# leonlang/simple_raytracer

Measured on AMD Instinct MI355X. Metric: Mrays/sec (primary+shadow) at 1920x1080; max per-pixel |dRGB| vs CPU ref, higher is better.
Workload: dtype f32; 1 GPU; ground_bunny: stanford-bunny (69,451 tris) over a ground slab, BVH + slab-AABB, 1920x1080, 1 light sample(s) [BASELINE.json configs[2]]; nodes=24216, tris=69463, parallelism=1 GPU, launch=hipGraph replay, 4 stream(s), pipeline=k_trace_nq+k_shade_tile

## Files before the change

simple_raytracer_amd/csrc/srt_hip.hip:

```cpp
#include <hip/hip_runtime.h>

#include <cfloat>
#include <cmath>
#include <cstdio>
#include <cstdlib>
#include <cstring>
#include <algorithm>
#include <array>
#include <atomic>
#include <deque>
#include <map>
#include <memory>
#include <new>
#include <thread>
#include <type_traits>
#include <vector>

#include "../../include/srt.h"
#include "srt_device.h"

using namespace srt;

#include "srt_kernels.h"
#include "srt_packet.h"
// ... 945 lines not shown

uint64_t srt_scene_device_bytes(const srt_scene* s) { return s ? s->bytes : 0; }
const char* srt_scene_pipeline(const srt_scene* s) { return s ? s->pipeline : ""; }
double srt_scene_overlap_estimate(const srt_scene* s) { return s ? s->rec->overlap : 0.; }

enum Variant : uint32_t {
    V_SHIPPED = 0,
    V_REFERENCE = 1,
    V_TRI_QUEUE = 2,
    V_NQ_TINY = 3,
    V_NQ_EXACT = 4,
    V_NQ_8X4 = 5,
    V_NQ_TINY_FILTER = 6,
    V_UNFUSED = 10,
    V_FUSED_5_WAVES = 11,
    V_FUSED_ROOTS_AGAIN = 12,
    V_FUSED_HALF = 13,
    V_FUSED_HALF_TINY = 14,
    V_FUSED_HALF_1024 = 15,
    V_FUSED_HALF_32_RAYS = 16,
    V_FUSED_64_RAYS = 17,
    V_XCD_ROWS = 18,
    V_FUSED_HALF_6_WAVES = 19,
    V_CHUNKED = 20,
    V_NQ_PK = 21,
    V_PK_PK = 22,
    V_PK_NQ = 23,
    V_NO_PACKET = 24,
    V_PK_WINDOWS = 25,
    V_COARSE_GRID = 27,
    V_TRACE_SHADE = 28,
    V_PK_ENTRY_ORDER = 29,
    V_FUSED_HALF_8_WAVES = 30,
    V_CAMERA_PK = 35,
    V_ROUND2_FORM = 40,
    V_ALL_WIDE = 41,
    V_ALL_NARROW = 42,
    V_LANE_ORDER = 43,
    V_GENERAL_SHADE = 44,
    V_ROOT_LOOP = 45,
    V_NO_UNION_BOX = 46,
    V_WIDE_STEP_COUNTERS = 47,
    V_HIT_6_WAVES = 53,
    V_FUSED_6_WAVES = 54,
    V_PK_AHEAD = 55,
    V_PK_AHEAD_SKIP = 56,
    V_PK_PLAIN = 57,
    V_PK_CLOCKS = 58,
    V_FUSED_FOUR_WAVES = 59,
    V_SHADOW_PLAIN_ROWS = 62,
    V_EXACT_TONE = 63,
    V_FULL_GRID = 64,
    V_HALF_7_WAVES = 65,
    V_HALF_8_WAVES_256 = 66,
};
static inline uint32_t variant_of(const srt_params* p) { return (p->flags >> 8) & 0xffu; }
static inline uint32_t variant_or_shipped(const srt_params* p) { const uint32_t v = variant_of(p); return v >= V_FULL_GRID && v <= V_HALF_8_WAVES_256 ? (uint32_t)V_SHIPPED : v; }
static inline bool shipped_choice(uint32_t v) {
    return v == V_SHIPPED || v == V_NO_PACKET || v == V_PK_WINDOWS || v == V_COARSE_GRID || v == V_PK_ENTRY_ORDER || v == V_CAMERA_PK ||
           (v >= V_ROUND2_FORM && v <= V_SHADOW_PLAIN_ROWS) || v == V_EXACT_TONE;
}

using RefHitFn = decltype(&k_closest_hit<false>);
using RefShadeFn = decltype(&k_shade<false>);
using QHitFn = decltype(&k_closest_hit_q<false>);
using NqHitFn = decltype(&k_closest_hit_nq<false, 512, 2, 2, true>);
using PkHitFn = decltype(&k_closest_hit_pk<false, true, false>);
using TraceFn = decltype(&k_trace_nq<false, 512, true, 7, 16>);
using TraceShadeFn = decltype(&k_trace_shade_nq<512, true, 6, 16>);
using ShadowPkFn = decltype(&k_shadow_pk<false, true, false>);
using ShadowNqFn = decltype(&k_shadow_nq<false, 512, true, 16, 6>);
using ShadeTileFn = decltype(&k_shade_tile<0>);
using TraceSpansFn = decltype(&k_trace_nq_spans<512, true, 7, 16>);
using ShadeTileSpansFn = decltype(&k_shade_tile_spans<0>);


enum BatchState { NOT_BATCHED, BATCH_FITS, BATCH_OTHER_SIZE };
enum Hold { HOLD_NONE, HOLD_FUSED, HOLD_PK };

struct SceneFacts {
    bool prefer_packet, int_shin, normals; double overlap; uint64_t bytes; uint32_t n_cu;
    uint32_t heavy_steps, pk_units, pk_take;
    uint32_t n_objects; const float* root_min; const float* root_max; uint32_t box_epoch;
};
static SceneFacts scene_facts(const srt_scene* s) {
    static const auto env = [](const char* name, uint32_t dflt) { const char* e = std::getenv(name); return e ? (uint32_t)std::strtoul(e, nullptr, 10) : dflt; };
    static const uint32_t heavy_steps = env("SRT_HEAVY_STEPS", 64u);
    static const uint32_t pk_units = env("SRT_PK_UNITS", 64u), pk_take = env("SRT_PK_TAKE", 4u);
    const bool boxes_known = s->rec->root_boxes_valid && !s->rec->boxes_change_in_replays;
    return SceneFacts{s->rec->prefer_packet, s->rec->int_shin, s->dev.tri_normals != nullptr, s->rec->overlap, s->bytes, (uint32_t)s->n_cu,
// ... 69 lines not shown
    if (holdable && (fused ? !pl.xcd_rows && !cam : pk_shadow)) {
        pl.hold = fused ? HOLD_FUSED : HOLD_PK;
        if (!fused) { pl.heavy_steps = f.heavy_steps; pl.pk_take = f.pk_take ? f.pk_take : 1u; pl.pk_units = 0u; }
        std::snprintf(pl.pipeline, sizeof(pl.pipeline), fused ? "k_trace_nq+k_shade_tile (batched)" : "k_closest_hit_nq+k_shadow_pk+k_shade_tile (batched)");
        return pl;
    }
    if (pk_shadow && v == V_SHIPPED && !count && !in_flight && batch == NOT_BATCHED) pl.heavy_steps = f.heavy_steps;

    #define NQ_HIT(CAP, TWL, THL, FILTER) do { \
        if (count) pl.nq_hit = &k_closest_hit_nq<true, CAP, TWL, THL, FILTER>; else pl.nq_hit = &k_closest_hit_nq<false, CAP, TWL, THL, FILTER>; \
        pl.grid_hit = dim3((wl + (2u << TWL) - 1) / (2u << TWL), (rows + (2u << THL) - 1) / (2u << THL)); } while (0)
    pl.grid_hit = grid8;
    switch (v) {
    case V_TRI_QUEUE:
        if (count) pl.q_hit = &k_closest_hit_q<true>; else pl.q_hit = &k_closest_hit_q<false>;
        pl.grid_hit = grid16; break;
    case V_NQ_TINY:        NQ_HIT(160, 2, 2, false); break;
    case V_NQ_EXACT:       NQ_HIT(512, 2, 2, false); break;
    case V_NQ_TINY_FILTER: NQ_HIT(160, 2, 2, true); break;
    case V_NQ_8X4:         NQ_HIT(1024, 3, 2, false); break;
    case V_UNFUSED:        NQ_HIT(512, 2, 2, true); break;
    default:
        if (pk_closest) {
            const bool xcd = pl.xcd_rows && !cam && !count;
            if (cam && count)  pl.pk_hit = &k_closest_hit_pk<true, true, false, true>;
            else if (cam)      pl.pk_hit = &k_closest_hit_pk<false, true, false, true>;
            else if (count)    pl.pk_hit = &k_closest_hit_pk<true, true, false>;
            else if (xcd)      pl.pk_hit = &k_closest_hit_pk<false, true, true>;
            else               pl.pk_hit = &k_closest_hit_pk<false, true, false>;
            pl.grid_hit = dim3((grid8.x + 1) / 2, xcd ? xcd_pad((grid8.y + 1) / 2) : (grid8.y + 1) / 2);
        } else if (fused && v == V_TRACE_SHADE && !count && !pl.xcd_rows && L < 64) {
            pl.trace_shade = &k_trace_shade_nq<512, true, 6, 16>;
        } else if (fused) {
            const bool half_tile = (v == V_SHIPPED && in_flight) || v == V_FUSED_HALF;
            const bool half_eight = (v == V_SHIPPED && in_flight && variant_of(p) != V_HALF_7_WAVES) || v == V_FUSED_HALF_8_WAVES;
            if (cam_nq)                        pl.trace = &k_trace_nq<false, 512, true, 5, 16, false, false, true>;
            else if (count)                    pl.trace = &k_trace_nq<true, 512, true, 5, 16>;
            else if (v == V_FUSED_5_WAVES)     pl.trace = &k_trace_nq<false, 512, true, 5, 16>;
            else if (v == V_FUSED_ROOTS_AGAIN) pl.trace = &k_trace_nq<false, 512, true, 6, 16, false, true>;
            else if (v == V_FUSED_64_RAYS)     pl.trace = &k_trace_nq<false, 512, true, 5, 64>;
            else if (v == V_FUSED_6_WAVES)     pl.trace = &k_trace_nq<false, 512, true, 6, 16>;
            else if (v == V_ALL_WIDE)          pl.trace = &k_trace_nq<false, 512, true, 6, 16, false, false, false, true>;
            else if (pl.xcd_rows)            { pl.trace = &k_trace_nq<false, 512, true, 6, 16, true>; pl.grid_hit.y = xcd_pad(grid8.y); }
            else if (v == V_FUSED_HALF_TINY) { pl.trace = &k_trace_nq_half<160, true, 6, 16>; pl.block_hit = 128; }
            else if (v == V_FUSED_HALF_1024) { pl.trace = &k_trace_nq_half<1024, true, 5, 16>; pl.block_hit = 128; }
            else if (v == V_FUSED_HALF_32_RAYS) { pl.trace = &k_trace_nq_half<512, true, 6, 32>; pl.block_hit = 128; }
            else if (v == V_FUSED_HALF_6_WAVES) { pl.trace = &k_trace_nq_half<512, true, 6, 16>; pl.block_hit = 128; }
            else if (half_eight && variant_of(p) == V_HALF_8_WAVES_256) { pl.trace = &k_trace_nq_half8<256, true, 16>; pl.block_hit = 128; }
            else if (half_eight)             { pl.trace = &k_trace_nq_half8<384, true, 16>; pl.block_hit = 128; }
            else if (half_tile)              { pl.trace = &k_trace_nq_half<512, true, 7, 16>; pl.block_hit = 128; }
            else                               pl.trace = &k_trace_nq<false, 512, true, 7, 16>;
        } else if (!count && v == V_COARSE_GRID) {
            pl.nq_hit = &k_closest_hit_nq<false, 512, 2, 2, true, true>;
            pl.grid_hit = dim3((grid8.x + 1) / 2, (grid8.y + 1) / 2);
        } else if (!count && v == V_ALL_WIDE) {
            pl.nq_hit = &k_closest_hit_nq<false, 512, 2, 2, true, false, true>;
        } else if (!count && v != V_HIT_6_WAVES) {
            pl.nq_hit = &k_closest_hit_nq<false, 512, 2, 2, true, false, false, 7>;
        } else {
            NQ_HIT(512, 2, 2, true);
        }
    }
    #undef NQ_HIT
    if (pk_shadow) {
        const uint64_t max_units = (uint64_t)n_tiles * 4u * 2u * ((L + 7) / 8);
        pl.grid_shadow = dim3((uint32_t)(max_units / 4 + 1 < (uint64_t)f.n_cu * 8 ? max_units / 4 + 1 : (uint64_t)f.n_cu * 8));
        if (count)                       pl.shadow_pk = &k_shadow_pk<true, true, false>;
        else if (v == V_PK_ENTRY_ORDER)  pl.shadow_pk = &k_shadow_pk<false, true, false, true>;
        else if (v == V_PK_AHEAD)        pl.shadow_pk = &k_shadow_pk<false, true, false, false, 1>;
        else if (v == V_PK_AHEAD_SKIP)   pl.shadow_pk = &k_shadow_pk<false, true, false, false, 2>;
        else if (pl.heavy_steps)         pl.shadow_pk = &k_shadow_pk<false, true, false, false, 0, true>;
        else if (v == V_PK_CLOCKS)       pl.shadow_pk = &k_shadow_pk<false, true, false, false, -1>;
        else if (v == V_PK_PLAIN)        pl.shadow_pk = &k_shadow_pk<false, true, false, false, 0>;
        else if (v == V_PK_WINDOWS)      pl.shadow_pk = &k_shadow_pk<false, true, true>;
        else                             pl.shadow_pk = &k_shadow_pk<false, true, false>;
    } else if (L && !fused) {
        pl.shadow_xcd_rows = v == V_SHADOW_PLAIN_ROWS ? 0u : pl.xcd_rows;
        if (chunked) pl.l_chunk = L / 4 > 4 ? (L + 3) / 4 : 4;
        pl.grid_shadow = dim3(grid8.x, pl.shadow_xcd_rows ? xcd_pad(grid8.y) : grid8.y, chunked ? (L + pl.l_chunk - 1) / pl.l_chunk : 1);
        if (chunked)                                       pl.shadow_nq = &k_shadow_nq<false, 512, true, 64, 6>;
        else if (count)                                    pl.shadow_nq = &k_shadow_nq<true, 512, false>;
        else if (v == V_NQ_TINY)                           pl.shadow_nq = &k_shadow_nq<false, 160, false>;
        else if (v == V_NQ_TINY_FILTER)                    pl.shadow_nq = &k_shadow_nq<false, 160, true>;
        else if (v == V_NQ_EXACT)                          pl.shadow_nq = &k_shadow_nq<false, 512, false>;
        else if (v == V_ROUND2_FORM || v == V_ALL_NARROW)  pl.shadow_nq = &k_shadow_nq<false, 512, true, 16, 6, false>;
        else                                               pl.shadow_nq = &k_shadow_nq<false, 512, true, 16, 6>;
    }
    if (pl.trace_shade) { std::snprintf(pl.pipeline, sizeof(pl.pipeline), "k_trace_shade_nq"); return pl; }
    if (f.int_shin && v != V_GENERAL_SHADE) pl.shade_tile = &k_shade_tile<1>; else pl.shade_tile = &k_shade_tile<0>;
    if (pl.trace && v == V_SHIPPED && !full_grid && !cam && !count && !pl.xcd_rows && !p->block_cols && p->block_stride == 1 && p->block_first == 0 &&
        p->spp == 1 && batch == NOT_BATCHED && f.root_min && wl == p->width && rows == p->height &&
        tile_spans(f.root_min, f.root_max, f.n_objects, p->width, p->height, (int)(-(float)p->width / 2), (int)(-(float)p->height / 2), p->focal, &pl.spans))
    {
        pl.spans.epoch = f.box_epoch;
        if (pl.block_hit == 128) pl.trace_spans = &k_trace_nq_half_spans<512, true, 7, 16>; else pl.trace_spans = &k_trace_nq_spans<512, true, 7, 16>;
        if (pl.trace == &k_trace_nq_half8<384, true, 16>) pl.trace_spans = &k_trace_nq_half8_spans<384, true, 16>;
        if (pl.trace == &k_trace_nq_half8<256, true, 16>) pl.trace_spans = &k_trace_nq_half8_spans<256, true, 16>;
        if (pl.shade_tile == &k_shade_tile<1>) pl.shade_tile_spans = &k_shade_tile_spans<1>; else pl.shade_tile_spans = &k_shade_tile_spans<0>;
        pl.grid_hit_full = grid8;
        pl.grid_hit = dim3(tile_spans_max_n(pl.spans), pl.spans.n_rows);
    } else {
        pl.spans.on = 0u;
    }
    std::snprintf(pl.pipeline, sizeof(pl.pipeline), "%s%s+k_shade_tile", fused ? "k_trace_nq" : (pk_closest ? "k_closest_hit_pk" : "k_closest_hit_nq"),
                  fused || !L ? "" : (pk_shadow ? "+k_shadow_pk" : "+k_shadow_nq"));
    return pl;
}

struct FrameParams {
    DevParams hit, shadow, shade;
    void sub_pixel(float x, float y) { hit.sub_x = shadow.sub_x = shade.sub_x = x; hit.sub_y = shadow.sub_y = shade.sub_y = y; }
};
static FrameParams dev_params(const srt_scene* s, const srt_params* p, const FramePlan& pl) {
    DevParams dp;
    dp.smooth = (p->flags & SRT_FLAG_SMOOTH_NORMALS) ? 1u : 0u; dp.shadow_px_major = 0u;
    dp.cam = p->ray_matrix ? 1u : 0u;
    for (int c = 0; c < 4; c++) for (int r3 = 0; r3 < 3; r3++) dp.cm[c * 3 + r3] = p->ray_matrix ? p->ray_matrix[c * 4 + r3] : 0.0f;
    dp.W = srt_cols_owned(p); dp.Wimg = p->width; dp.col_block = p->block_cols; dp.H = p->height; dp.rows = srt_rows_owned(p);
    dp.block_rows = p->block_rows; dp.block_first = p->block_first; dp.block_stride = p->block_stride;
    dp.i0 = (int)(-(float)p->width / 2); dp.j0 = (int)(-(float)p->height / 2);
    dp.sub_x = 0.0f; dp.sub_y = 0.0f;
    dp.focal = p->focal; dp.n_lights = p->n_lights; dp.lights = s->d_lights;
    dp.shadow_div = p->shadow_div; dp.reinhard = p->reinhard; dp.gamma = p->gamma;
    dp.bg = (uint32_t)p->background[0] | ((uint32_t)p->background[1] << 8) | ((uint32_t)p->background[2] << 16);
    dp.xcd_rows = pl.xcd_rows; dp.exp = pl.exp; dp.heavy_steps = pl.heavy_steps; dp.pk_units = pl.pk_units; dp.pk_take = pl.pk_take;
    FrameParams fp{dp, dp, dp};
    fp.shadow.xcd_rows = pl.shadow_xcd_rows; fp.shade.shadow_px_major = pl.shadow_px_major;
    return fp;
}

struct BatchCollector {
    std::vector<FrameItem> items;
    std::vector<FrameItem> items_pk;
// ... 1434 lines not shown
```

simple_raytracer_amd/csrc/srt_kernels.h:

```cpp
#pragma once
#include <hip/hip_runtime.h>
#include <stdint.h>
#include <type_traits>

#include "srt_device.h"
#include "srt_tile_spans.h"

using namespace srt;

struct DevScene {
    const DevNode* nodes;
    const DevWide* wide;
    const int32_t* obj_root_info;
    const DevNode* root_nodes;
    const float* scene_box;
    const DevTri* tris;
    const DevTriO* tris_o;
    const int32_t* tri_obj;
    const int32_t* tri_tex;
    const float* tri_tc;
    const float* tri_normals;
    const float* obj_color;
    const float* obj_mat;
    const int2* obj_range;
// ... 299 lines not shown
    }
}
template <typename DRAIN>
__device__ __forceinline__ void leaf_queue_push2(uint32_t* tq, uint32_t& tqn, bool lane_order, uint32_t info_a, bool leaf_a, uint32_t info_b, bool leaf_b,
                                                 uint32_t slot, DRAIN drain) {
    const unsigned long long ma = __ballot(leaf_a), mb = __ballot(leaf_b);
    if (ma | mb) {
        uint32_t pos = tqn + lane_prefix(ma) + lane_prefix(mb), q = pos + (leaf_a ? 1u : 0u);
        if (!lane_order) { pos = tqn + lane_prefix(ma); q = tqn + (uint32_t)__popcll(ma) + lane_prefix(mb); }
        if (leaf_a) { tq[2 * pos] = info_a; tq[2 * pos + 1] = slot; }
        if (leaf_b) { tq[2 * q] = info_b; tq[2 * q + 1] = slot; }
        tqn += (uint32_t)__popcll(ma) + (uint32_t)__popcll(mb);
        __builtin_amdgcn_wave_barrier();
        while (tqn >= 64) drain();
    }
}


#ifdef SRT_DIAG
#define SRT_STAMP(v) do { v = __builtin_amdgcn_s_memtime(); __builtin_amdgcn_s_waitcnt(0xC07F); } while (0)
__device__ __forceinline__ void diag_tile_record(float* rgb_linear, uint32_t bx, uint32_t by, uint32_t gx, unsigned long long k0, unsigned long long k1,
                                                 unsigned long long ka = 0, unsigned long long kb = 0) {
    if ((threadIdx.x & 63) == 0 && rgb_linear) {
        unsigned long long* dgp = reinterpret_cast<unsigned long long*>(rgb_linear) + (((size_t)by * gx + bx) * 4 + (threadIdx.x >> 6)) * 8;
        const unsigned long long hw = __builtin_amdgcn_s_getreg((31 << 11) | 4), xcc = __builtin_amdgcn_s_getreg((3 << 11) | 20);
        dgp[5] = hw | (xcc << 32); dgp[6] = k0; dgp[7] = k1;
        if (ka) { dgp[3] = ka - k0; dgp[4] = kb - ka; }
    }
}
#else
#define SRT_STAMP(v) do { } while (0)
#endif

template <bool COUNT, int NQCAP, int TWL, int THL, bool FILTER, bool CAM = false, bool WIDE = false, bool HALF = false>
__device__ __forceinline__ void closest_hit_phase(const DevScene& s, const DevParams& p, uint32_t* nq, uint32_t* tq,
                                                  unsigned long long* best, float4* dir,
                                                  int32_t* __restrict__ hit_id, float* __restrict__ t_out,
                                                  float* __restrict__ rgb_linear, uint8_t* __restrict__ rgb8,
                                                  unsigned long long* __restrict__ counters, int32_t& out_id, float& out_t, V3& out_d,
                                                  const uint32_t bx, const uint32_t by, const uint32_t gx,
                                                  const uint32_t wave,
                                                  uint32_t* __restrict__ qcount = nullptr, uint32_t* __restrict__ qlist = nullptr, uint32_t qcap = 0,
                                                  const uint32_t* root_pass = nullptr) {
    constexpr int P = 1 << (TWL + THL);
    const uint32_t lane = threadIdx.x & 63;
    const float4* nodes4 = reinterpret_cast<const float4*>(s.nodes);
    const float4* tris4 = reinterpret_cast<const float4*>(s.tris);
    static_assert(!HALF || (TWL == 3 && THL == 2), "a half tile is 8x4 pixels");
    const uint32_t tile_x = HALF ? bx * 8 + ((lane >> 4) & 1u) * 4 : (bx * 2 + (wave & 1)) << TWL, tile_r = HALF ? by * 8 + wave * 4 : (by * 2 + (wave >> 1)) << THL;
    const uint32_t px = tile_x + (lane & (HALF ? 3u : (1u << TWL) - 1)), r = tile_r + ((lane >> (HALF ? 2 : TWL)) & ((1u << THL) - 1));
    const bool live = lane < P && pixel_live(p, px, r);
    const V3 o = CAM ? ray_origin(p) : mk(0.0f, 0.0f, 0.0f);
    if (lane < P) {
        V3 dmine = mk(0.f, 0.f, p.focal);
        best[lane] = ~0ull;
        if (live) dmine = primary_dir(p, px, image_row(p, r));
        if (CAM) dir[lane] = make_float4(dmine.x, dmine.y, dmine.z, 0.f);
        else { const RayRcp rq = ray_rcp(dmine); dir[lane] = make_float4(dmine.x, dmine.y, rq.x, rq.y); }
    }
    const float rcp_focal = __builtin_amdgcn_rcpf(p.focal);
    const unsigned long long livem = __ballot(live);
    unsigned long long n_node = 0, n_tri = 0;
    uint32_t nqn = 0, tqn = 0;
    __builtin_amdgcn_wave_barrier();
    unsigned long long dg_pop = 0, dg_load = 0; (void)dg_pop; (void)dg_load;
    unsigned long long dg_t0 = 0, dg_a = 0, dg_b = 0, dg_test = 0, dg_commit = 0, dg_tri = 0, dg_steps = 0, dg_batches = 0, dg_items = 0, dg_titems = 0;
    (void)dg_t0; (void)dg_a; (void)dg_b; (void)dg_test; (void)dg_commit; (void)dg_tri; (void)dg_steps; (void)dg_batches; (void)dg_items; (void)dg_titems;
    SRT_STAMP(dg_t0);

    auto tri_batch = [&]() {
        const uint32_t m = tqn < 64 ? tqn : 64;
        tqn -= m;
#ifdef SRT_DIAG
        unsigned long long c0, c1; SRT_STAMP(c0); dg_batches++; dg_titems += m;
#endif
        const uint32_t sh = m <= 8 ? 3u : (m <= 16 ? 2u : (m <= 32 ? 1u : 0u));
        const uint32_t S = 1u << sh, pi = lane >> sh, sub = lane & (S - 1u);
// ... 117 lines not shown
                    end = in_r ? s.nodes[rnode].skip : rnode;
                    hop = (in_l && in_r) ? rnode : -1;
                }
                while (__ballot(i < end)) {
                    int32_t inf2 = -1;
                    bool lp2 = false;
                    if (i < end) {
                        if (i == hop) i = hop + 1;
                        else {
                            const float4 a = nodes4[2 * (size_t)i], b = nodes4[2 * (size_t)i + 1];
                            const int32_t sk = __float_as_int(b.z);
                            inf2 = __float_as_int(b.w);
                            if (COUNT) n_node++;
                            if (ray_aabb_nb(o, d, a.x, a.y, a.z, a.w, b.x, b.y)) {
                                lp2 = inf2 >= 0 && (inf2 & LEAF_MAX) != 0;
                                i = i + 1;
                            } else {
                                i = sk;
                            }
                        }
                    }
                    leaf_queue_push2(tq, tqn, p.exp & 1u, (uint32_t)inf2, lp2, 0u, false, pl, tri_batch);
                }
            }
            __builtin_amdgcn_wave_barrier();
#ifdef SRT_DIAG
            { unsigned long long c2_; SRT_STAMP(c2_); dg_commit += (c2_ - dg_b) - (dg_tri - tri_before); }
#endif
        }
    }
    } else
    for (uint32_t obj0 = 0; obj0 < n_obj && nlive; obj0 += OBJ_G) {
        const uint32_t g = (n_obj - obj0) < OBJ_G ? (n_obj - obj0) : OBJ_G;
        if (!COUNT && root_pass) {
            for (uint32_t base = 0; base < P * g; base += 64) {
                const uint32_t k = base + lane_again(lane);
                const uint32_t pl = k & (P - 1), ob = k >> (TWL + THL);
                const bool ok = k < P * g && ((livem >> pl) & 1ull) && ((root_pass[pl] >> (obj0 + ob)) & 1u);
                int32_t root = 0, info = -1;
                if (ok) { root = s.obj_range[obj0 + ob].x; info = s.root_nodes[obj0 + ob].leaf; }
                const bool inner = ok && info < 0, leafp = ok && info >= 0 && (info & LEAF_MAX) != 0;
                const unsigned long long im = __ballot(inner);
                if (inner) {
                    uint32_t pos = nqn + 2 * lane_prefix(im), pos1 = pos + 1;
                    if (!(p.exp & 1u)) { pos = nqn + lane_prefix(im); pos1 = pos + (uint32_t)__popcll(im); }
                    nq[pos] = ((uint32_t)(~info) << 6) | pl;
                    nq[pos1] = ((uint32_t)(root + 1) << 6) | pl;
                }
                nqn += 2 * (uint32_t)__popcll(im);
                leaf_queue_push(tq, tqn, (uint32_t)info, leafp, pl, tri_batch);
            }
        } else
        for (uint32_t base = 0; base < P * g; base += 64) {
            const uint32_t k = base + lane_again(lane);
            const uint32_t pl = k & (P - 1), ob = k >> (TWL + THL);
            const bool ok = k < P * g && ((livem >> pl) & 1ull);
            const unsigned long long m = __ballot(ok);
            if (ok) nq[nqn + lane_prefix(m)] = ((uint32_t)s.obj_range[obj0 + ob].x << 6) | pl;
            nqn += (uint32_t)__popcll(m);
        }
        __builtin_amdgcn_wave_barrier();
        while (nqn) {
            const uint32_t m = nqn < 64 ? nqn : 64;
            nqn -= m;
#ifdef SRT_DIAG
            SRT_STAMP(dg_a); dg_steps++; dg_items += m;
            const unsigned long long tri_before = dg_tri;
// ... 770 lines not shown
                                                   unsigned long long* __restrict__ counters, uint32_t l_chunk = 0xffffffffu) {
    __shared__ uint32_t nq_all[4][NQCAP];
    __shared__ uint32_t tq_all[4][LQ_WORDS];
    __shared__ ShadowLds<RS> lds_all[4];
    const uint32_t lane = threadIdx.x & 63, wave = threadIdx.x >> 6;
    const uint32_t gx = gridDim.x;
    uint32_t bx = blockIdx.x, by = blockIdx.y;
    if (p.xcd_rows) {
        const uint32_t w = blockIdx.y * gx + blockIdx.x, idx = w >> 3;
        by = (idx / gx) * 8u + (w & 7u); bx = idx % gx;
        if (by >= (p.rows + 7u) / 8u) return;
    }
    const uint32_t px = bx * 8 + (wave & 1) * 4 + (lane & 3), r = by * 8 + (wave >> 1) * 4 + ((lane >> 2) & 3);
    int32_t id = -1; float t = 0.f;
    V3 d = mk(0.f, 0.f, p.focal);
    if (lane < NQ_P && pixel_live(p, px, r)) { id = hit_id[(size_t)r * p.W + px]; t = t_in[(size_t)r * p.W + px]; d = primary_dir(p, px, image_row(p, r)); }
    const uint32_t l_begin = l_chunk == 0xffffffffu ? 0u : blockIdx.z * l_chunk;
    shadow_phase<SEQ, NQCAP, FILTER, RS, true, WIDE>(s, p, nq_all[wave], tq_all[wave], lds_all[wave], id, t, d, shadow_bits, counters, bx, by, gx, wave,
                                         l_begin, l_chunk == 0xffffffffu ? 0xffffffffu : l_begin + l_chunk);
}

template <bool INT_SHIN = false, typename SH>
__device__ __forceinline__ void shade_hit_pixel(const DevScene& s, const DevParams& p, const int32_t id, const float t, const uint32_t px, const uint32_t r,
                                                SH shadowed, float* __restrict__ rgb_linear, uint8_t* __restrict__ rgb8) {
    const V3 o = ray_origin(p);
    const V3 d = primary_dir(p, px, image_row(p, r));
    const Surface f = surface_at(s, id, o, d, t, p.smooth != 0u);
    V3 sum = mk(0.0f, 0.0f, 0.0f);
    add_light_samples<INT_SHIN>(sum, f, o, d, t, p.lights, 0u, p.n_lights, p.shadow_div, shadowed);
    store_pixel(rgb_linear, rgb8, (size_t)r * p.W + px, sum, true, p.reinhard, p.gamma, p.bg, p.exp);
}

template <bool COUNT, int NQCAP, bool FILTER, int RS, bool XCD_ROWS, bool ROOTS_AGAIN, bool SHADE = false, bool CAM = false, bool WIDE = false, bool ROW_Z = false,
          bool HALF = false>
__device__ __forceinline__ void trace_nq_body(const DevScene& s, const DevParams& p, int32_t* __restrict__ hit_id, float* __restrict__ t_out,
                                              float* __restrict__ rgb_linear, uint8_t* __restrict__ rgb8,
                                              unsigned long long* __restrict__ shadow_bits, unsigned long long* __restrict__ counters,
                                              unsigned long long* __restrict__ counters_next = nullptr, uint32_t* __restrict__ qcount = nullptr,
                                              const TileSpans* spans = nullptr,
                                              const uint32_t* __restrict__ box_epoch = nullptr) {
    uint32_t span_bx = blockIdx.x, span_by = blockIdx.y; bool span_on = false;
    if (spans) {
        if (!box_epoch) {
            uint32_t row0 = spans->row0;
            uint32_t sp = reinterpret_cast<const uint32_t*>(spans->row)[blockIdx.y < TILE_SPAN_ROWS ? blockIdx.y : TILE_SPAN_ROWS - 1u];
            asm volatile("" : "+s"(sp), "+s"(row0));
            if (blockIdx.x >= (sp >> 16)) return;
            span_on = true;
            span_by = row0 + blockIdx.y;
            span_bx = (sp & 0xffffu) + blockIdx.x;
        } else {
            uint32_t sp = reinterpret_cast<const uint32_t*>(spans->row)[blockIdx.y < TILE_SPAN_ROWS ? blockIdx.y : TILE_SPAN_ROWS - 1u];
            uint32_t n_rows = spans->n_rows;
            asm volatile("" : "+s"(sp), "+s"(n_rows));
            const bool outside = blockIdx.y >= n_rows || blockIdx.x - (sp & 0xffffu) >= (sp >> 16);
            if (outside && *box_epoch == spans->epoch) return;
        }
    }
    __shared__ uint32_t fin_count;
    __shared__ int32_t fin_id[64];
    __shared__ float fin_t[64];
    if (SHADE) {
        if (threadIdx.x == 0) fin_count = 0u;
        if (counters_next) zero_next_counters(counters_next);
        if (qcount && blockIdx.x == 0 && blockIdx.y == 0) for (uint32_t i = threadIdx.x; i < (uint32_t)QL_COUNTERS; i += 256u) qcount[i * QL_STRIDE] = 0u;
    }
    static_assert(!HALF || (!SHADE && !COUNT), "the half-tile form has no one-launch and no counting build");
    constexpr int NW = HALF ? 2 : 4, P = HALF ? 32 : NQ_P;
    __shared__ uint32_t nq_all[NW][NQCAP];
    __shared__ uint32_t tq_all[NW][LQ_WORDS];
    const uint32_t wave = threadIdx.x >> 6;
    ShadowLds<RS, P>* L;
    int32_t id; float t; V3 d;
    unsigned long long k0 = 0, k1 = 0; (void)k0; (void)k1;
    SRT_STAMP(k0);
    const uint32_t gx = span_on ? (p.W + 7u) / 8u : gridDim.x;
    uint32_t bx = span_bx, by = ROW_Z ? blockIdx.z : span_by;
    if (XCD_ROWS) {
        const uint32_t w = blockIdx.y * gx + blockIdx.x, idx = w >> 3;
        by = (idx / gx) * 8u + (w & 7u); bx = idx % gx;
        if (by >= (p.rows + 7u) / 8u) return;
    }
    __shared__ uint32_t root_pass[64];
    const bool roots_done = !COUNT && !ROOTS_AGAIN && s.n_objects <= 32u;
    unsigned long long ka = 0, kb = 0; (void)ka; (void)kb;
    ShadowLds<RS, P>* lds_tile = nullptr;
    if constexpr (HALF) {
        __shared__ HalfTileLds<RS, P> half_all[NW];
        using Shadow = ShadowLds<RS, P>;
        static_assert(sizeof(half_all[0].closest) <= offsetof(Shadow, mask), "dir[] and best[] end at or before the root masks that wait in ShadowLds::mask");
        static_assert(sizeof(HalfTileLds<RS, P>) == sizeof(Shadow) && sizeof(Shadow) % 4 == 0, "the stride between the two waves' masks is counted in words");
        if (finish_background_tile<FILTER, CAM>(s, p, hit_id, t_out, rgb_linear, rgb8, shadow_bits, bx, by, gx, half_all[0].shadow.mask, sizeof(HalfTileLds<RS, P>) / 4)) return;
        SRT_STAMP(ka);
        closest_hit_phase<COUNT, NQCAP, 3, 2, FILTER, CAM, WIDE, true>(s, p, nq_all[wave], tq_all[wave], half_all[wave].closest.best, half_all[wave].closest.dir,
                                                                 hit_id, t_out, rgb_linear, rgb8, counters, id, t, d, bx, by, gx, wave, nullptr, nullptr, 0,
                                                                 roots_done ? half_all[wave].shadow.mask : nullptr);
        L = &half_all[wave].shadow;
        __builtin_amdgcn_fence(__ATOMIC_ACQ_REL, "wavefront");
    } else {
    __shared__ unsigned long long best_all[NW][P];
    __shared__ float4 dir_all[NW][P];
    __shared__ ShadowLds<RS, P> lds_all[NW];
    if (!COUNT && finish_background_tile<FILTER, CAM>(s, p, hit_id, t_out, rgb_linear, rgb8, shadow_bits, bx, by, gx, root_pass)) return;
    SRT_STAMP(ka);
    closest_hit_phase<COUNT, NQCAP, 2, 2, FILTER, CAM, WIDE>(s, p, nq_all[wave], tq_all[wave], best_all[wave], dir_all[wave],
                                                       hit_id, t_out, rgb_linear, rgb8, counters, id, t, d, bx, by, gx, wave, nullptr, nullptr, 0,
                                                       roots_done ? root_pass + wave * 16 : nullptr);
    L = &lds_all[wave]; lds_tile = lds_all;
    }
    __builtin_amdgcn_wave_barrier();
    SRT_STAMP(kb);
    shadow_phase<COUNT, NQCAP, FILTER, RS, true, WIDE, P>(s, p, nq_all[wave], tq_all[wave], *L, id, t, d, shadow_bits, counters, bx, by, gx, wave);
#ifdef SRT_DIAG
    SRT_STAMP(k1); diag_tile_record(rgb_linear, bx, by, gx, k0, k1, ka, kb);
#endif
    if (SHADE) {
        const uint32_t lane = threadIdx.x & 63;
        if (lane < NQ_P) { fin_id[wave * NQ_P + lane] = id; fin_t[wave * NQ_P + lane] = t; }
        __builtin_amdgcn_fence(__ATOMIC_RELEASE, "workgroup");
        uint32_t before = 0;
        if (lane == 0) before = atomicAdd(&fin_count, 1u);
        before = __builtin_amdgcn_readfirstlane(before);
        if (before != 3u) return;
        __builtin_amdgcn_fence(__ATOMIC_ACQUIRE, "workgroup");
        const uint32_t q = lane >> 4, pl = lane & 15u;
        const uint32_t px = bx * 8 + (q & 1u) * 4 + (pl & 3u), r = by * 8 + (q >> 1) * 4 + (pl >> 2);
        const int32_t hid = fin_id[lane];
        if (hid >= 0 && pixel_live(p, px, r)) {
            const uint32_t* mask = lds_tile[q].mask;
            shade_hit_pixel(s, p, hid, fin_t[lane], px, r, [&](uint32_t l) -> bool { return (mask[l] >> pl) & 1u; }, rgb_linear, rgb8);
        }
    }
}

template <bool COUNT, int NQCAP, bool FILTER, int MINW, int RS, bool XCD_ROWS = false, bool ROOTS_AGAIN = false, bool CAM = false, bool WIDE = false>
__global__ __launch_bounds__(256, MINW) void k_trace_nq(DevScene s, DevParams p, int32_t* __restrict__ hit_id, float* __restrict__ t_out,
                                                  float* __restrict__ rgb_linear, uint8_t* __restrict__ rgb8,
                                                  unsigned long long* __restrict__ shadow_bits, unsigned long long* __restrict__ counters) {
    trace_nq_body<COUNT, NQCAP, FILTER, RS, XCD_ROWS, ROOTS_AGAIN, false, CAM, WIDE>(s, p, hit_id, t_out, rgb_linear, rgb8, shadow_bits, counters);
}
template <int NQCAP, bool FILTER, int MINW, int RS>
__global__ __launch_bounds__(128, MINW) void k_trace_nq_half(DevScene s, DevParams p, int32_t* __restrict__ hit_id, float* __restrict__ t_out,
                                                       float* __restrict__ rgb_linear, uint8_t* __restrict__ rgb8,
                                                       unsigned long long* __restrict__ shadow_bits, unsigned long long* __restrict__ counters) {
    trace_nq_body<false, NQCAP, FILTER, RS, false, false, false, false, false, false, true>(s, p, hit_id, t_out, rgb_linear, rgb8, shadow_bits, counters);
// ... 1 lines not shown
template <int NQCAP, bool FILTER, int MINW, int RS>
__global__ __launch_bounds__(256, MINW) void k_trace_nq_spans(DevScene s, DevParams p, int32_t* __restrict__ hit_id, float* __restrict__ t_out,
                                                        float* __restrict__ rgb_linear, uint8_t* __restrict__ rgb8,
                                                        unsigned long long* __restrict__ shadow_bits, unsigned long long* __restrict__ counters,
                                                        const uint32_t* __restrict__ box_epoch, const TileSpans spans) {
    trace_nq_body<false, NQCAP, FILTER, RS, false, false>(s, p, hit_id, t_out, rgb_linear, rgb8, shadow_bits, counters, nullptr, nullptr, &spans, box_epoch);
}
template <int NQCAP, bool FILTER, int MINW, int RS>
__global__ __launch_bounds__(128, MINW) void k_trace_nq_half_spans(DevScene s, DevParams p, int32_t* __restrict__ hit_id, float* __restrict__ t_out,
                                                             float* __restrict__ rgb_linear, uint8_t* __restrict__ rgb8,
                                                             unsigned long long* __restrict__ shadow_bits, unsigned long long* __restrict__ counters,
                                                             const uint32_t* __restrict__ box_epoch, const TileSpans spans) {
    trace_nq_body<false, NQCAP, FILTER, RS, false, false, false, false, false, false, true>(s, p, hit_id, t_out, rgb_linear, rgb8, shadow_bits, counters, nullptr, nullptr, &spans, box_epoch);
}
#if defined(__HIP_DEVICE_COMPILE__)
#define SRT_NO_PACKED_F32 __attribute__((target("no-packed-fp32-ops")))
#else
#define SRT_NO_PACKED_F32
#endif
template <int NQCAP, bool FILTER, int RS>
__global__ __launch_bounds__(128, 8) SRT_NO_PACKED_F32
void k_trace_nq_half8(DevScene s, DevParams p, int32_t* __restrict__ hit_id, float* __restrict__ t_out,
                      float* __restrict__ rgb_linear, uint8_t* __restrict__ rgb8,
                      unsigned long long* __restrict__ shadow_bits, unsigned long long* __restrict__ counters) {
    trace_nq_body<false, NQCAP, FILTER, RS, false, false, false, false, false, false, true>(s, p, hit_id, t_out, rgb_linear, rgb8, shadow_bits, counters);
}
template <int NQCAP, bool FILTER, int RS>
__global__ __launch_bounds__(128, 8) SRT_NO_PACKED_F32
void k_trace_nq_half8_spans(DevScene s, DevParams p, int32_t* __restrict__ hit_id, float* __restrict__ t_out,
                            float* __restrict__ rgb_linear, uint8_t* __restrict__ rgb8,
                            unsigned long long* __restrict__ shadow_bits, unsigned long long* __restrict__ counters,
                            const uint32_t* __restrict__ box_epoch, const TileSpans spans) {
    trace_nq_body<false, NQCAP, FILTER, RS, false, false, false, false, false, false, true>(s, p, hit_id, t_out, rgb_linear, rgb8, shadow_bits, counters, nullptr, nullptr, &spans, box_epoch);
}
template <int NQCAP, bool FILTER, int MINW, int RS, bool XCD_ROWS = false>
__global__ __launch_bounds__(256, MINW) void k_trace_shade_nq(DevScene s, DevParams p, int32_t* __restrict__ hit_id, float* __restrict__ t_out,
                                                        float* __restrict__ rgb_linear, uint8_t* __restrict__ rgb8,
                                                        unsigned long long* __restrict__ counters, unsigned long long* __restrict__ counters_next,
                                                        uint32_t* __restrict__ qcount) {
    trace_nq_body<false, NQCAP, FILTER, RS, XCD_ROWS, false, true>(s, p, hit_id, t_out, rgb_linear, rgb8, nullptr, counters, counters_next, qcount);
}

struct FrameItem {
    DevScene s; DevParams p;
    int32_t* hit_id; float* t_out; float* rgb_linear; uint8_t* rgb8;
    unsigned long long* shadow_bits; unsigned long long* counters; unsigned long long* counters_next; uint32_t* qcount;
    uint32_t* qlist; uint32_t qcap, pad_;
};
static_assert(sizeof(FrameItem) == sizeof(DevScene) + sizeof(DevParams) + 9 * 8 + 8, "FrameItem has no implicit padding");
constexpr uint32_t FRAME_TAB_MAX = 36;
struct FrameTab { FrameItem it[FRAME_TAB_MAX]; };
static_assert(sizeof(FrameTab) <= 16384, "the frame table is copied into the kernel-argument segment at every launch");
template <int NQCAP, bool FILTER, bool ROW_Z = false>
__global__ __launch_bounds__(256, 7) void k_closest_hit_nq_batch(const FrameTab tab) {
    const FrameItem& it = tab.it[ROW_Z ? blockIdx.y : blockIdx.z];
    const uint32_t tile_row = ROW_Z ? blockIdx.z : blockIdx.y;
    __shared__ uint32_t nq_all[4][NQCAP];
    __shared__ uint32_t tq_all[4][LQ_WORDS];
    __shared__ unsigned long long best_all[4][NQ_P];
    __shared__ float4 dir_all[4][NQ_P];
    __shared__ uint32_t root_pass[64];
    const uint32_t wave = threadIdx.x >> 6;
    int32_t id; float t; V3 d;
    const bool roots_done = it.s.n_objects <= 32u;
    if (finish_background_tile<FILTER>(it.s, it.p, it.hit_id, it.t_out, it.rgb_linear, it.rgb8, nullptr, blockIdx.x, tile_row, gridDim.x, root_pass)) return;
    closest_hit_phase<false, NQCAP, 2, 2, FILTER, false, false>(it.s, it.p, nq_all[wave], tq_all[wave], best_all[wave], dir_all[wave],
// ... 514 lines not shown
```

Measured before the change: 38790 Mrays/s.

## Add one-wave-per-workgroup half-tile trace kernel with XCD-paired block order

Adds a k_trace_nq_wave8_spans kernel in which each 64-thread workgroup runs one half tile. Each wave does its own root pass instead of sharing one across a two-wave block, which removes cross-wave coupling and per-block LDS sharing and lets waves schedule independently. An optional XCD_PAIRS block-index remap places the two halves of a tile in adjacent groups of eight blocks, so they likely land on the same XCD for L2 locality. It becomes the default when the half8 kernel is selected and L<=4. The cost is duplicated root traversal per wave, a skipped background-tile shortcut, and more, smaller workgroups.

New measurement: 40240 Mrays/s, median of 6. 1.04x the previous value.

```diff
diff --git a/simple_raytracer_amd/csrc/srt_hip.hip b/simple_raytracer_amd/csrc/srt_hip.hip
--- a/simple_raytracer_amd/csrc/srt_hip.hip
+++ b/simple_raytracer_amd/csrc/srt_hip.hip
@@ -1001,6 +1001,8 @@
     V_TRACE_SHADE = 28,
     V_PK_ENTRY_ORDER = 29,
     V_FUSED_HALF_8_WAVES = 30,
+    V_WAVE_8 = 31,
+    V_WAVE_8_ADJACENT = 32,
     V_CAMERA_PK = 35,
     V_ROUND2_FORM = 40,
     V_ALL_WIDE = 41,
@@ -1022,9 +1024,10 @@
     V_FULL_GRID = 64,
     V_HALF_7_WAVES = 65,
     V_HALF_8_WAVES_256 = 66,
+    V_HALF_8_TWO_WAVES = 67,
 };
 static inline uint32_t variant_of(const srt_params* p) { return (p->flags >> 8) & 0xffu; }
-static inline uint32_t variant_or_shipped(const srt_params* p) { const uint32_t v = variant_of(p); return v >= V_FULL_GRID && v <= V_HALF_8_WAVES_256 ? (uint32_t)V_SHIPPED : v; }
+static inline uint32_t variant_or_shipped(const srt_params* p) { const uint32_t v = variant_of(p); return (v >= V_FULL_GRID && v <= V_HALF_8_TWO_WAVES) || v == V_WAVE_8 || v == V_WAVE_8_ADJACENT ? (uint32_t)V_SHIPPED : v; }
 static inline bool shipped_choice(uint32_t v) {
     return v == V_SHIPPED || v == V_NO_PACKET || v == V_PK_WINDOWS || v == V_COARSE_GRID || v == V_PK_ENTRY_ORDER || v == V_CAMERA_PK ||
            (v >= V_ROUND2_FORM && v <= V_SHADOW_PLAIN_ROWS) || v == V_EXACT_TONE;
@@ -1160,8 +1163,9 @@
         } else if (fused && v == V_TRACE_SHADE && !count && !pl.xcd_rows && L < 64) {
             pl.trace_shade = &k_trace_shade_nq<512, true, 6, 16>;
         } else if (fused) {
-            const bool half_tile = (v == V_SHIPPED && in_flight) || v == V_FUSED_HALF;
-            const bool half_eight = (v == V_SHIPPED && in_flight && variant_of(p) != V_HALF_7_WAVES) || v == V_FUSED_HALF_8_WAVES;
+            const bool hinted = in_flight || variant_of(p) == V_WAVE_8;
+            const bool half_tile = (v == V_SHIPPED && hinted) || v == V_FUSED_HALF;
+            const bool half_eight = (v == V_SHIPPED && hinted && variant_of(p) != V_HALF_7_WAVES) || v == V_FUSED_HALF_8_WAVES;
             if (cam_nq)                        pl.trace = &k_trace_nq<false, 512, true, 5, 16, false, false, true>;
             else if (count)                    pl.trace = &k_trace_nq<true, 512, true, 5, 16>;
             else if (v == V_FUSED_5_WAVES)     pl.trace = &k_trace_nq<false, 512, true, 5, 16>;
@@ -1224,9 +1228,16 @@
         if (pl.block_hit == 128) pl.trace_spans = &k_trace_nq_half_spans<512, true, 7, 16>; else pl.trace_spans = &k_trace_nq_spans<512, true, 7, 16>;
         if (pl.trace == &k_trace_nq_half8<384, true, 16>) pl.trace_spans = &k_trace_nq_half8_spans<384, true, 16>;
         if (pl.trace == &k_trace_nq_half8<256, true, 16>) pl.trace_spans = &k_trace_nq_half8_spans<256, true, 16>;
+        const bool one_wave = pl.trace == &k_trace_nq_half8<384, true, 16> && variant_of(p) != V_HALF_8_TWO_WAVES &&
+                              (L <= 4 || variant_of(p) == V_WAVE_8 || variant_of(p) == V_WAVE_8_ADJACENT);
+        const bool xcd_pairs = one_wave && variant_of(p) != V_WAVE_8_ADJACENT;
+        if (one_wave) { pl.trace_spans = &k_trace_nq_wave8_spans<384, true, 16, false>; pl.block_hit = 64; }
+        if (xcd_pairs) pl.trace_spans = &k_trace_nq_wave8_spans<384, true, 16, true>;
         if (pl.shade_tile == &k_shade_tile<1>) pl.shade_tile_spans = &k_shade_tile_spans<1>; else pl.shade_tile_spans = &k_shade_tile_spans<0>;
         pl.grid_hit_full = grid8;
         pl.grid_hit = dim3(tile_spans_max_n(pl.spans), pl.spans.n_rows);
+        if (xcd_pairs) { pl.grid_hit_full.x = (pl.grid_hit_full.x + 7u) / 8u * 8u; pl.grid_hit.x = (pl.grid_hit.x + 7u) / 8u * 8u; }
+        if (one_wave) { pl.grid_hit_full.x *= 2u; pl.grid_hit.x *= 2u; }
     } else {
         pl.spans.on = 0u;
     }
diff --git a/simple_raytracer_amd/csrc/srt_kernels.h b/simple_raytracer_amd/csrc/srt_kernels.h
--- a/simple_raytracer_amd/csrc/srt_kernels.h
+++ b/simple_raytracer_amd/csrc/srt_kernels.h
@@ -355,7 +355,7 @@
 #define SRT_STAMP(v) do { } while (0)
 #endif
 
-template <bool COUNT, int NQCAP, int TWL, int THL, bool FILTER, bool CAM = false, bool WIDE = false, bool HALF = false>
+template <bool COUNT, int NQCAP, int TWL, int THL, bool FILTER, bool CAM = false, bool WIDE = false, bool HALF = false, bool OWN_ROOTS = false>
 __device__ __forceinline__ void closest_hit_phase(const DevScene& s, const DevParams& p, uint32_t* nq, uint32_t* tq,
                                                   unsigned long long* best, float4* dir,
                                                   int32_t* __restrict__ hit_id, float* __restrict__ t_out,
@@ -364,8 +364,10 @@
                                                   const uint32_t bx, const uint32_t by, const uint32_t gx,
                                                   const uint32_t wave,
                                                   uint32_t* __restrict__ qcount = nullptr, uint32_t* __restrict__ qlist = nullptr, uint32_t qcap = 0,
-                                                  const uint32_t* root_pass = nullptr) {
+                                                  const uint32_t* root_pass = nullptr,
+                                                  const bool own_roots = false) {
     constexpr int P = 1 << (TWL + THL);
+    static_assert(!OWN_ROOTS || (HALF && !WIDE && !COUNT), "the wave's own root pass is the half-tile form's, over the 32 B records");
     const uint32_t lane = threadIdx.x & 63;
     const float4* nodes4 = reinterpret_cast<const float4*>(s.nodes);
     const float4* tris4 = reinterpret_cast<const float4*>(s.tris);
@@ -549,7 +551,36 @@
     } else
     for (uint32_t obj0 = 0; obj0 < n_obj && nlive; obj0 += OBJ_G) {
         const uint32_t g = (n_obj - obj0) < OBJ_G ? (n_obj - obj0) : OBJ_G;
-        if (!COUNT && root_pass) {
+        if (OWN_ROOTS && own_roots) {
+            for (uint32_t base = 0; base < P * g; base += 64) {
+                const uint32_t k = base + lane_again(lane);
+                const uint32_t pl = k & (P - 1), ob = k >> (TWL + THL);
+                bool ok = k < P * g && ((livem >> pl) & 1ull);
+                int32_t root = 0, info = -1;
+                if (ok) {
+                    const float4* rn = reinterpret_cast<const float4*>(s.root_nodes) + 2 * (size_t)(obj0 + ob);
+                    const float4 a = rn[0], b = rn[1];
+                    root = s.obj_range[obj0 + ob].x;
+                    const float4 dxy = dir[pl];
+                    const V3 d = mk(dxy.x, dxy.y, CAM ? dxy.z : p.focal);
+                    RayRcp rc;
+                    if (CAM) rc = ray_rcp(d);
+                    else { rc.x = dxy.z; rc.y = dxy.w; rc.z = __builtin_fmaf(dxy.z, 0.0f, rcp_focal); }
+                    info = __float_as_int(b.w);
+                    ok = slab_pass<FILTER>(o, d, rc, a.x, a.y, a.z, a.w, b.x, b.y);
+                }
+                const bool inner = ok && info < 0, leafp = ok && info >= 0 && (info & LEAF_MAX) != 0;
+                const unsigned long long im = __ballot(inner);
+                if (inner) {
+                    uint32_t pos = nqn + 2 * lane_prefix(im), pos1 = pos + 1;
+                    if (!(p.exp & 1u)) { pos = nqn + lane_prefix(im); pos1 = pos + (uint32_t)__popcll(im); }
+                    nq[pos] = ((uint32_t)(~info) << 6) | pl;
+                    nq[pos1] = ((uint32_t)(root + 1) << 6) | pl;
+                }
+                nqn += 2 * (uint32_t)__popcll(im);
+                leaf_queue_push(tq, tqn, (uint32_t)info, leafp, pl, tri_batch);
+            }
+        } else if (!COUNT && root_pass) {
             for (uint32_t base = 0; base < P * g; base += 64) {
                 const uint32_t k = base + lane_again(lane);
                 const uint32_t pl = k & (P - 1), ob = k >> (TWL + THL);
@@ -1386,14 +1417,35 @@
 }
 
 template <bool COUNT, int NQCAP, bool FILTER, int RS, bool XCD_ROWS, bool ROOTS_AGAIN, bool SHADE = false, bool CAM = false, bool WIDE = false, bool ROW_Z = false,
-          bool HALF = false>
+          bool HALF = false, int ONE = 0>
 __device__ __forceinline__ void trace_nq_body(const DevScene& s, const DevParams& p, int32_t* __restrict__ hit_id, float* __restrict__ t_out,
                                               float* __restrict__ rgb_linear, uint8_t* __restrict__ rgb8,
                                               unsigned long long* __restrict__ shadow_bits, unsigned long long* __restrict__ counters,
                                               unsigned long long* __restrict__ counters_next = nullptr, uint32_t* __restrict__ qcount = nullptr,
                                               const TileSpans* spans = nullptr,
                                               const uint32_t* __restrict__ box_epoch = nullptr) {
+    static_assert(!ONE || HALF, "one wave per workgroup is a half tile");
     uint32_t span_bx = blockIdx.x, span_by = blockIdx.y; bool span_on = false;
+    if constexpr (ONE != 0) {
+        const uint32_t blk_x = ONE == 2 ? ((blockIdx.x >> 4) << 3) | (blockIdx.x & 7u) : blockIdx.x >> 1;
+        if (ONE == 2 && blk_x >= (p.W + 7u) / 8u) return;
+        span_bx = blk_x;
+        if (!box_epoch) {
+            uint32_t row0 = spans->row0;
+            uint32_t sp = reinterpret_cast<const uint32_t*>(spans->row)[blockIdx.y < TILE_SPAN_ROWS ? blockIdx.y : TILE_SPAN_ROWS - 1u];
+            asm volatile("" : "+s"(sp), "+s"(row0));
+            if (blk_x >= (sp >> 16)) return;
+            span_on = true;
+            span_by = row0 + blockIdx.y;
+            span_bx = (sp & 0xffffu) + blk_x;
+        } else {
+            uint32_t sp = reinterpret_cast<const uint32_t*>(spans->row)[blockIdx.y < TILE_SPAN_ROWS ? blockIdx.y : TILE_SPAN_ROWS - 1u];
+            uint32_t n_rows = spans->n_rows;
+            asm volatile("" : "+s"(sp), "+s"(n_rows));
+            const bool outside = blockIdx.y >= n_rows || blk_x - (sp & 0xffffu) >= (sp >> 16);
+            if (outside && *box_epoch == spans->epoch) return;
+        }
+    } else
     if (spans) {
         if (!box_epoch) {
             uint32_t row0 = spans->row0;
@@ -1420,15 +1472,17 @@
         if (qcount && blockIdx.x == 0 && blockIdx.y == 0) for (uint32_t i = threadIdx.x; i < (uint32_t)QL_COUNTERS; i += 256u) qcount[i * QL_STRIDE] = 0u;
     }
     static_assert(!HALF || (!SHADE && !COUNT), "the half-tile form has no one-launch and no counting build");
-    constexpr int NW = HALF ? 2 : 4, P = HALF ? 32 : NQ_P;
+    static_assert(!ONE || (!XCD_ROWS && !ROW_Z && !CAM && !ROOTS_AGAIN), "one wave per workgroup: the plain tile order of a frame with spans only");
+    constexpr int NW = ONE ? 1 : HALF ? 2 : 4, P = HALF ? 32 : NQ_P;
     __shared__ uint32_t nq_all[NW][NQCAP];
     __shared__ uint32_t tq_all[NW][LQ_WORDS];
-    const uint32_t wave = threadIdx.x >> 6;
+    const uint32_t wave = ONE == 2 ? (blockIdx.x >> 3) & 1u : ONE ? blockIdx.x & 1u : threadIdx.x >> 6;
+    const uint32_t wq = ONE ? 0u : wave;
     ShadowLds<RS, P>* L;
     int32_t id; float t; V3 d;
     unsigned long long k0 = 0, k1 = 0; (void)k0; (void)k1;
     SRT_STAMP(k0);
-    const uint32_t gx = span_on ? (p.W + 7u) / 8u : gridDim.x;
+    const uint32_t gx = ONE ? (p.W + 7u) / 8u : span_on ? (p.W + 7u) / 8u : gridDim.x;
     uint32_t bx = span_bx, by = ROW_Z ? blockIdx.z : span_by;
     if (XCD_ROWS) {
         const uint32_t w = blockIdx.y * gx + blockIdx.x, idx = w >> 3;
@@ -1444,12 +1498,20 @@
         using Shadow = ShadowLds<RS, P>;
         static_assert(sizeof(half_all[0].closest) <= offsetof(Shadow, mask), "dir[] and best[] end at or before the root masks that wait in ShadowLds::mask");
         static_assert(sizeof(HalfTileLds<RS, P>) == sizeof(Shadow) && sizeof(Shadow) % 4 == 0, "the stride between the two waves' masks is counted in words");
+        if constexpr (ONE) {
+            if (by * 8u + wave * 4u >= p.rows) return;
+            SRT_STAMP(ka);
+            closest_hit_phase<COUNT, NQCAP, 3, 2, FILTER, CAM, WIDE, true, true>(s, p, nq_all[0], tq_all[0], half_all[0].closest.best, half_all[0].closest.dir,
+                                                                           hit_id, t_out, rgb_linear, rgb8, counters, id, t, d, bx, by, gx, wave, nullptr, nullptr, 0,
+                                                                           nullptr, roots_done);
+        } else {
         if (finish_background_tile<FILTER, CAM>(s, p, hit_id, t_out, rgb_linear, rgb8, shadow_bits, bx, by, gx, half_all[0].shadow.mask, sizeof(HalfTileLds<RS, P>) / 4)) return;
         SRT_STAMP(ka);
         closest_hit_phase<COUNT, NQCAP, 3, 2, FILTER, CAM, WIDE, true>(s, p, nq_all[wave], tq_all[wave], half_all[wave].closest.best, half_all[wave].closest.dir,
                                                                  hit_id, t_out, rgb_linear, rgb8, counters, id, t, d, bx, by, gx, wave, nullptr, nullptr, 0,
                                                                  roots_done ? half_all[wave].shadow.mask : nullptr);
-        L = &half_all[wave].shadow;
+        }
+        L = &half_all[wq].shadow;
         __builtin_amdgcn_fence(__ATOMIC_ACQ_REL, "wavefront");
     } else {
     __shared__ unsigned long long best_all[NW][P];
@@ -1464,7 +1526,7 @@
     }
     __builtin_amdgcn_wave_barrier();
     SRT_STAMP(kb);
-    shadow_phase<COUNT, NQCAP, FILTER, RS, true, WIDE, P>(s, p, nq_all[wave], tq_all[wave], *L, id, t, d, shadow_bits, counters, bx, by, gx, wave);
+    shadow_phase<COUNT, NQCAP, FILTER, RS, true, WIDE, P>(s, p, nq_all[wq], tq_all[wq], *L, id, t, d, shadow_bits, counters, bx, by, gx, wave);
 #ifdef SRT_DIAG
     SRT_STAMP(k1); diag_tile_record(rgb_linear, bx, by, gx, k0, k1, ka, kb);
 #endif
@@ -1532,6 +1594,14 @@
                             unsigned long long* __restrict__ shadow_bits, unsigned long long* __restrict__ counters,
                             const uint32_t* __restrict__ box_epoch, const TileSpans spans) {
     trace_nq_body<false, NQCAP, FILTER, RS, false, false, false, false, false, false, true>(s, p, hit_id, t_out, rgb_linear, rgb8, shadow_bits, counters, nullptr, nullptr, &spans, box_epoch);
+}
+template <int NQCAP, bool FILTER, int RS, bool XCD_PAIRS = false>
+__global__ __launch_bounds__(64, 8) SRT_NO_PACKED_F32
+void k_trace_nq_wave8_spans(DevScene s, DevParams p, int32_t* __restrict__ hit_id, float* __restrict__ t_out,
+                            float* __restrict__ rgb_linear, uint8_t* __restrict__ rgb8,
+                            unsigned long long* __restrict__ shadow_bits, unsigned long long* __restrict__ counters,
+                            const uint32_t* __restrict__ box_epoch, const TileSpans spans) {
+    trace_nq_body<false, NQCAP, FILTER, RS, false, false, false, false, false, false, true, XCD_PAIRS ? 2 : 1>(s, p, hit_id, t_out, rgb_linear, rgb8, shadow_bits, counters, nullptr, nullptr, &spans, box_epoch);
 }
 template <int NQCAP, bool FILTER, int MINW, int RS, bool XCD_ROWS = false>
 __global__ __launch_bounds__(256, MINW) void k_trace_shade_nq(DevScene s, DevParams p, int32_t* __restrict__ hit_id, float* __restrict__ t_out,
```
